# tdavchev/DESIRE

Measured on AMD Instinct MI355X. Metric: agent-trajectory-samples/sec (K=20, T_pred=40), higher is better.
Workload: dtype f32; 1 GPU; BASELINE configs[1]: SDD-like synthetic windows, 32 agent slots/window, K=20, T_obs=8/T_pred=40, H=128, L=128, fp32, posterior CVAE, IOC 1 refinement, social grid 4x4, scene grid 64x64x32; 512 windows/step/GPU; windows_per_gpu=512, rows_per_gpu=327680, parallelism=scene-sharded x1

## Files before the change

### desire_amd/csrc/kernels_conv.hip

```cpp
#include "common.h"
#include "kernels.h"

__global__ __launch_bounds__(DS_WG) void k_conv1(ConvArgs a) {
    __shared__ __attribute__((aligned(16))) float in_s[36 * 40];
    const int n = blockIdx.x, tid = threadIdx.x;
    DYN_N(a, n, n)
    for (int i = tid; i < 36 * 40; i += DS_WG) in_s[i] = 0.f;
    __syncthreads();
    for (int i = tid; i < 1024; i += DS_WG) in_s[((i >> 5) + 1) * 40 + (i & 31) + 1] = a.in[(size_t)n * 1024 + i];
    const int co = tid & 31, pg = tid >> 5;
    float wr[25];
#pragma unroll
    for (int k = 0; k < 25; ++k) wr[k] = a.w_raw[k * 32 + co];
    __syncthreads();
    const float sc = a.scale[co], sh = a.shift[co];
    for (int p = pg; p < 256; p += 8) {
        const int oy = p >> 4, ox = p & 15;
        const int base = (2 * ox) & ~3;
        const bool odd = ox & 1;
        float acc = 0.f;
#pragma unroll
        for (int ky = 0; ky < 5; ++ky) {
            const float* row = in_s + (2 * oy + ky) * 40 + base;
            const float4 v0 = *reinterpret_cast<const float4*>(row), v1 = *reinterpret_cast<const float4*>(row + 4);
            const float t0 = odd ? v0.z : v0.x, t1 = odd ? v0.w : v0.y, t2 = odd ? v1.x : v0.z, t3 = odd ? v1.y : v0.w, t4 = odd ? v1.z : v1.x;
            acc = fmaf(t0, wr[ky * 5 + 0], acc);
            acc = fmaf(t1, wr[ky * 5 + 1], acc);
            acc = fmaf(t2, wr[ky * 5 + 2], acc);
            acc = fmaf(t3, wr[ky * 5 + 3], acc);
            acc = fmaf(t4, wr[ky * 5 + 4], acc);
        }
        { const size_t ix = ((size_t)n * 256 + p) * 32 + co; a.out[ix] = conv_epilogue(acc, sc, sh, a.mode, false, a.yprev, ix); }
    }
}
void launch_conv1(const ConvArgs& a, hipStream_t s) {
    hipLaunchKernelGGL(k_conv1, dim3(a.n), dim3(DS_WG), 0, s, a);
}

template <int CI, int IW, int OW, int STRIDE, int PAD, int CO>
__global__ __launch_bounds__(DS_WG) void k_conv_gather(ConvArgs a) {
    constexpr int PIX = OW * OW, SPW = DS_TM / PIX, LDP = CI + 4, NT = CO / 32, G = CI / 8;
    constexpr int MT = (NT == 4) ? 2 : 1;
    extern __shared__ __attribute__((aligned(16))) float smem[];
    float* zero_row = smem;
    float* in_s = smem + LDP;
    const int lane = lane_id(), w = wave_id(), tid = threadIdx.x;
    const int s0 = blockIdx.x * SPW;
    DYN_N(a, n, s0)
    for (int i = tid; i < LDP; i += DS_WG) zero_row[i] = 0.f;
    constexpr int Q = CI / 4;
    auto pos = [](int y, int x) {
        if (STRIDE == 2) return (((y & 1) * 2 + (x & 1)) * (IW / 2) + (y >> 1)) * (IW / 2) + (x >> 1);
        return y * IW + x;
    };
    for (int i = tid; i < SPW * IW * IW * Q; i += DS_WG) {
        const int pix = i / Q, c4 = i - pix * Q;
        const int ls = pix / (IW * IW), pp = pix - ls * IW * IW;
        const int smp = s0 + ls;
        float4 v = make_float4(0.f, 0.f, 0.f, 0.f);
        if (smp < a.n) v = *reinterpret_cast<const float4*>(a.in + ((size_t)s0 * IW * IW + pix) * CI + c4 * 4);
        *reinterpret_cast<float4*>(in_s + (ls * IW * IW + pos(pp / IW, pp % IW)) * LDP + c4 * 4) = v;
    }
    __syncthreads();
    const int nt = (NT == 4) ? w : (w & 1);
    const int mt0 = (NT == 4) ? 0 : (w >> 1);
    f32x16 acc[MT];
    int oy[MT], ox[MT], sm[MT];
#pragma unroll
    for (int m = 0; m < MT; ++m) {
        acc[m] = zero16();
        const int r = (mt0 + m) * 32 + (lane & 31);
        sm[m] = r / PIX;
        const int q = r - sm[m] * PIX;
        oy[m] = q / OW;
        ox[m] = q - oy[m] * OW;
    }
    for (int ky = 0; ky < 5; ++ky)
        for (int kx = 0; kx < 5; ++kx) {
            const float* ap[MT];
#pragma unroll
            for (int m = 0; m < MT; ++m) {
                const int iy = oy[m] * STRIDE + ky - PAD, ix = ox[m] * STRIDE + kx - PAD;
                const bool ok = iy >= 0 && iy < IW && ix >= 0 && ix < IW;
                ap[m] = (ok ? in_s + (sm[m] * IW * IW + pos(iy, ix)) * LDP : zero_row) + 4 * (lane >> 5);
            }
            mma_groups_ptr<MT>(acc, ap, a.Wp + ((size_t)((ky * 5 + kx) * NT + nt) * G) * 64 + lane, G);
        }
    const int co = nt * 32 + (lane & 31);
    const float sc = a.scale[co], sh = a.shift[co];
#pragma unroll
    for (int m = 0; m < MT; ++m)
#pragma unroll
        for (int i = 0; i < 16; ++i) {
            const int r = (mt0 + m) * 32 + acc_row(i);
            const int smp = s0 + r / PIX;
            if (smp < a.n) { const size_t ix = ((size_t)s0 * PIX + r) * CO + co; a.out[ix] = conv_epilogue(acc[m][i], sc, sh, a.mode, false, a.yprev, ix); }
        }
}
void launch_conv2(const ConvArgs& a, hipStream_t s) {
    const size_t lds = (36 + 256 * 36) * sizeof(float);
    hipLaunchKernelGGL((k_conv_gather<32, 16, 8, 2, 1, 64>), dim3(a.n), dim3(DS_WG), lds, s, a);
}
void launch_conv3(const ConvArgs& a, hipStream_t s) {
    const size_t lds = (68 + 4 * 64 * 68) * sizeof(float);
    launch_big_lds<k_conv_gather<64, 8, 4, 1, 0, 128>>(dim3((a.n + 3) / 4), dim3(DS_WG), lds, s, a);
}

template <bool FWD>
__global__ __launch_bounds__(DS_WG) void k_deconv2(ConvArgs a) {
    extern __shared__ __attribute__((aligned(16))) float out_s[];
    const int lane = lane_id(), w = wave_id();
    const int hf = w & 1, sp = w >> 1;
    asm volatile("" ::: "a255");
    DYN_N(a, n, blockIdx.x * 4)
    for (int bx = blockIdx.x; bx * 4 < a.n; bx += gridDim.x) {
        const int s0 = bx * 4 + sp * 2;
        const int c = lane & 31, hi = lane >> 5;
        float O[8][8];
    #pragma unroll
        for (int oy = 0; oy < 8; ++oy)
    #pragma unroll
            for (int ox = 0; ox < 8; ++ox) O[oy][ox] = 0.f;
        float4 af[16];
        {
            const int row = lane & 31;
            const int smp = min(s0 + ((row >> 2) & 1), a.n - 1);
            const float* src = a.in + ((size_t)smp * 16 + (row >> 3) * 4 + (row & 3)) * 128 + 4 * hi;
    #pragma unroll
            for (int g = 0; g < 16; ++g) af[g] = *reinterpret_cast<const float4*>(src + g * 8);
        }
        int woff = 0;
        asm volatile("" : "+s"(woff));
        const float4* wp = a.Wp + woff + lane;
        auto load_b = [&](float4 (&b)[8], int q) {
            const float4* bp = wp + ((size_t)((q >> 1) * 2 + hf) * 16 + (q & 1) * 8) * 64;
    #pragma unroll
            for (int g = 0; g < 8; ++g) b[g] = bp[g * 64];
        };
        float4 b[2][8];
        load_b(b[0], 0);
        f32x16 acc = zero16();
    #pragma unroll
        for (int q = 0; q < 50; ++q) {
            if (q + 1 < 50) load_b(b[(q + 1) & 1], q + 1);
            __builtin_amdgcn_sched_barrier(0);
            const float4 (&bt)[8] = b[q & 1];
            if (!(q & 1)) acc = zero16();
    #pragma unroll
            for (int g = 0; g < 8; ++g) {
                const float4 av = af[(q & 1) * 8 + g];
                acc = mfma32(av.x, bt[g].x, acc);
                acc = mfma32(av.y, bt[g].y, acc);
                acc = mfma32(av.z, bt[g].z, acc);
                acc = mfma32(av.w, bt[g].w, acc);
            }
            if (q & 1) {
                const int tap = q >> 1, ky = tap / 5, kx = tap - ky * 5;
    #pragma unroll
                for (int i = 0; i < 16; ++i) O[(i >> 2) + ky][(i & 3) + kx] = O[(i >> 2) + ky][(i & 3) + kx] + acc[i];
            }
            __builtin_amdgcn_sched_barrier(0);
        }
        float* my = out_s + (sp * 2) * 4096;
    #pragma unroll
        for (int o = 0; o < 64; ++o) my[(hi * 64 + o) * 64 + hf * 32 + c] = O[o >> 3][o & 7];
        const int er = lane >> 3, ec = hf * 32 + (lane & 7) * 4;
        const float4 sc4 = *reinterpret_cast<const float4*>(a.scale + ec), sh4 = *reinterpret_cast<const float4*>(a.shift + ec);
        for (int i = 0; i < 16; ++i) {
            const int sp_px = i * 8 + er;
            const int smp = s0 + (sp_px >> 6);
            if (smp < a.n) {
                const float4 v = *reinterpret_cast<const float4*>(my + sp_px * 64 + ec);
                const size_t ix = ((size_t)smp * 64 + (sp_px & 63)) * 64 + ec;
                float4 o;
                if (FWD) {
                    o.x = eluf_(v.x * sc4.x + sh4.x); o.y = eluf_(v.y * sc4.y + sh4.y);
                    o.z = eluf_(v.z * sc4.z + sh4.z); o.w = eluf_(v.w * sc4.w + sh4.w);
                } else {
                    o.x = conv_epilogue(v.x, sc4.x, sh4.x, a.mode, false, a.yprev, ix);
                    o.y = conv_epilogue(v.y, sc4.y, sh4.y, a.mode, false, a.yprev, ix + 1);
                    o.z = conv_epilogue(v.z, sc4.z, sh4.z, a.mode, false, a.yprev, ix + 2);
                    o.w = conv_epilogue(v.w, sc4.w, sh4.w, a.mode, false, a.yprev, ix + 3);
                }
                *reinterpret_cast<float4*>(a.out + ix) = o;
            }
        }
    }
}
void launch_deconv2(const ConvArgs& a, hipStream_t s) {
    const int ng = dyn_units(a.n, a.dyn);
    if (a.mode == 0) launch_big_lds<k_deconv2<true>>(dim3((ng + 3) / 4), dim3(DS_WG), 4 * 4096 * sizeof(float), s, a);
    else launch_big_lds<k_deconv2<false>>(dim3((ng + 3) / 4), dim3(DS_WG), 4 * 4096 * sizeof(float), s, a);
}

template <bool FWD, int NS>
__global__ __launch_bounds__(NS * 64) void k_deconv3(ConvArgs a) {
    constexpr int LDP = 68;
    extern __shared__ __attribute__((aligned(16))) float smem[];
    float* zero_row = smem;
    float* in_s = smem + 128;
    const int lane = lane_id(), w = wave_id(), tid = threadIdx.x;
    DYN_N(a, n, blockIdx.x * NS)
    for (int bx = blockIdx.x; bx * NS < a.n; bx += gridDim.x) {
        const int s0 = bx * NS;
        for (int i = tid; i < 128; i += NS * 64) zero_row[i] = 0.f;
        for (int i = tid; i < NS * 64 * 16; i += NS * 64) {
            const int pix = i >> 4, c4 = i & 15;
            const int smp = s0 + (pix >> 6);
            float4 v = make_float4(0.f, 0.f, 0.f, 0.f);
            if (smp < a.n) v = *reinterpret_cast<const float4*>(a.in + ((size_t)s0 * 64 + pix) * 64 + c4 * 4);
            *reinterpret_cast<float4*>(in_s + pix * LDP + c4 * 4) = v;
        }
        __syncthreads();
        const int smp = s0 + w;
        const float* mine = in_s + w * 64 * LDP;
        const int c = lane & 31, hi = lane >> 5;
        float4 sc[4], sh[4];
    #pragma unroll
        for (int q = 0; q < 4; ++q) {
            sc[q] = *reinterpret_cast<const float4*>(a.scale + 8 * q + 4 * hi);
            sh[q] = *reinterpret_cast<const float4*>(a.shift + 8 * q + 4 * hi);
        }
        int qy[2], qx[2];
    #pragma unroll
        for (int m = 0; m < 2; ++m) { const int q = m * 32 + (lane & 31); qy[m] = q >> 3; qx[m] = q & 7; }
        for (int py = 0; py < 2; ++py)
            for (int px = 0; px < 2; ++px) {
                f32x16 acc[2] = {zero16(), zero16()};
                for (int ky = 1 - py; ky < 5; ky += 2)
                    for (int kx = 1 - px; kx < 5; kx += 2) {
                        const int dy = (py + 1 - ky) / 2, dx = (px + 1 - kx) / 2;
                        const float* ap[2];
    #pragma unroll
                        for (int m = 0; m < 2; ++m) {
                            const int iy = qy[m] + dy, ix = qx[m] + dx;
                            const bool ok = iy >= 0 && iy < 8 && ix >= 0 && ix < 8;
                            ap[m] = (ok ? mine + (iy * 8 + ix) * LDP : zero_row + ((((w * 64 + iy * 8 + ix + 64) * LDP + 128) & 63))) + 4 * hi;
                        }
                        mma_groups_ptr<2, true>(acc, ap, a.Wp + ((size_t)(ky * 5 + kx) * 8) * 64 + lane, 8);
                    }
                if (smp < a.n) {
    #pragma unroll
                    for (int m = 0; m < 2; ++m) {
                        const int oy = 2 * qy[m] + py, ox = 2 * qx[m] + px;
                        const size_t base = ((size_t)smp * 256 + oy * 16 + ox) * 32 + 4 * hi;
    #pragma unroll
                        for (int q = 0; q < 4; ++q) {
                            const size_t ix = base + 8 * q;
                            float4 o;
                            if (FWD) {
                                o.x = eluf_(acc[m][4 * q] * sc[q].x + sh[q].x); o.y = eluf_(acc[m][4 * q + 1] * sc[q].y + sh[q].y);
                                o.z = eluf_(acc[m][4 * q + 2] * sc[q].z + sh[q].z); o.w = eluf_(acc[m][4 * q + 3] * sc[q].w + sh[q].w);
                            } else {
                                o.x = conv_epilogue(acc[m][4 * q], sc[q].x, sh[q].x, a.mode, false, a.yprev, ix);
                                o.y = conv_epilogue(acc[m][4 * q + 1], sc[q].y, sh[q].y, a.mode, false, a.yprev, ix + 1);
                                o.z = conv_epilogue(acc[m][4 * q + 2], sc[q].z, sh[q].z, a.mode, false, a.yprev, ix + 2);
                                o.w = conv_epilogue(acc[m][4 * q + 3], sc[q].w, sh[q].w, a.mode, false, a.yprev, ix + 3);
                            }
                            *reinterpret_cast<float4*>(a.out + ix) = o;
                        }
                    }
                }
            }
        __syncthreads();
    }
}
void launch_deconv3(const ConvArgs& a, hipStream_t s) {
    const size_t lds = (128 + (size_t)4 * 64 * 68) * sizeof(float);
    const int ng = dyn_units(a.n, a.dyn);
    if (a.mode == 0) launch_big_lds<k_deconv3<true, 4>>(dim3((ng + 3) / 4), dim3(256), lds, s, a);
    else launch_big_lds<k_deconv3<false, 4>>(dim3((ng + 3) / 4), dim3(256), lds, s, a);
}

__global__ __launch_bounds__(DS_WG) void k_deconv4(ConvArgs a) {
    constexpr int LDP = 36;
    __shared__ __attribute__((aligned(16))) float in_s[256 * LDP];
    __shared__ __attribute__((aligned(16))) float w_s[25 * 32];
    const int n = blockIdx.x, tid = threadIdx.x, lane = lane_id(), w = wave_id();
    for (int i = tid; i < 256 * 8; i += DS_WG) {
        const int pix = i >> 3, c4 = i & 7;
        *reinterpret_cast<float4*>(in_s + pix * LDP + c4 * 4) =
            *reinterpret_cast<const float4*>(a.in + ((size_t)n * 256 + pix) * 32 + c4 * 4);
    }
    for (int i = tid; i < 800; i += DS_WG) w_s[i] = a.w_raw[i];
    __syncthreads();
    const int py = w >> 1, px = w & 1;
    const float sc = a.scale[0], sh = a.shift[0];
    for (int j = 0; j < 4; ++j) {
        const int q = j * 64 + lane;
        const int qy = q >> 4, qx = q & 15;
        float acc = 0.f;
        for (int ky = 1 - py; ky < 5; ky += 2) {
            const int iy = qy + (py + 1 - ky) / 2;
            if (iy < 0 || iy >= 16) continue;
            for (int kx = 1 - px; kx < 5; kx += 2) {
                const int ix = qx + (px + 1 - kx) / 2;
                if (ix < 0 || ix >= 16) continue;
                const float* ip = in_s + (iy * 16 + ix) * LDP;
                const float* wp = w_s + (ky * 5 + kx) * 32;
#pragma unroll
                for (int c4 = 0; c4 < 8; ++c4) {
                    const float4 x = *reinterpret_cast<const float4*>(ip + c4 * 4);
                    const float4 ww = *reinterpret_cast<const float4*>(wp + c4 * 4);
                    acc = fmaf(x.x, ww.x, acc); acc = fmaf(x.y, ww.y, acc);
                    acc = fmaf(x.z, ww.z, acc); acc = fmaf(x.w, ww.w, acc);
                }
            }
        }
        { const size_t ix = (size_t)n * 1024 + (2 * qy + py) * 32 + 2 * qx + px; a.out[ix] = conv_epilogue(acc, sc, sh, a.mode, true, a.yprev, ix); }
    }
}
__global__ __launch_bounds__(DS_WG) void k_deconv4_tp(ConvArgs a) {
    __shared__ float xacc[4 * 1024];
    const int lane = lane_id(), w = wave_id(), tid = threadIdx.x;
    const int smp = blockIdx.x * 4 + w;
    DYN_N(a, n, blockIdx.x * 4)
    for (int i = tid; i < 4 * 1024; i += DS_WG) xacc[i] = 0.f;
    __syncthreads();
    float* xa = xacc + w * 1024;
    const float* __restrict__ wr = a.w_raw;
    if (smp < a.n) {
#pragma unroll 1
        for (int j = 0; j < 4; ++j) {
            const int p = j * 64 + lane, iy = p >> 4, ix = p & 15;
            float4 x[8];
            const float4* src = reinterpret_cast<const float4*>(a.in + ((size_t)smp * 256 + p) * 32);
#pragma unroll
            for (int c4 = 0; c4 < 8; ++c4) x[c4] = src[c4];
#pragma unroll 1
            for (int ky = 0; ky < 5; ++ky) {
                const int Y = 2 * iy + ky - 1;
#pragma unroll
                for (int kx = 0; kx < 5; ++kx) {
                    const float* wt = wr + (ky * 5 + kx) * 32;
                    float acc = 0.f;
#pragma unroll
                    for (int c4 = 0; c4 < 8; ++c4) {
                        acc = fmaf(x[c4].x, wt[c4 * 4], acc); acc = fmaf(x[c4].y, wt[c4 * 4 + 1], acc);
                        acc = fmaf(x[c4].z, wt[c4 * 4 + 2], acc); acc = fmaf(x[c4].w, wt[c4 * 4 + 3], acc);
                    }
                    const int X = 2 * ix + kx - 1;
                    if (Y >= 0 && Y < 32 && X >= 0 && X < 32) xa[Y * 32 + X] += acc;
                }
            }
        }
        const float sc = a.scale[0], sh = a.shift[0];
#pragma unroll
        for (int i = 0; i < 16; ++i) {
            const int o = i * 64 + lane;
            a.out[(size_t)smp * 1024 + o] = sigmoidf_(xa[o] * sc + sh);
        }
    }
}
void launch_deconv4(const ConvArgs& a, hipStream_t s) {
    if (a.mode == 0) hipLaunchKernelGGL(k_deconv4_tp, dim3((a.n + 3) / 4), dim3(DS_WG), 0, s, a);
    else hipLaunchKernelGGL(k_deconv4, dim3(a.n), dim3(DS_WG), 0, s, a);
}
```

### desire_amd/csrc/kernels_rnn.hip

```cpp
#include "common.h"
#include "kernels.h"
#include <cstdlib>
#include <map>
#include <tuple>

#define RNN_WG 512

__device__ __forceinline__ f32x16 splat16(float v) {
    f32x16 z;
#pragma unroll
    for (int i = 0; i < 16; ++i) z[i] = v;
    return z;
}

__device__ __forceinline__ void mma1(f32x16& acc, const float* a_lane, const float4* __restrict__ b_lane, int G) {
    f32x16 t[1] = {acc};
    mma_groups<1>(t, a_lane, 0, b_lane, G);
    acc = t[0];
}

template <int H, int TM, bool ROLL>
__device__ __forceinline__ void encoder_tile(const EncArgs& a, int blk) {
    extern __shared__ __attribute__((aligned(16))) float smem[];
    constexpr int LDH = H + 4, NT = H >> 5, G = H >> 3, NTHR = NT * (TM / 32) * 64;
    float* hs = smem;
    float* xs = smem + TM * LDH;
    const int lane = lane_id(), w = wave_id(), tid = threadIdx.x;
    const int cb = w % NT, mt = w / NT;
    const int A = a.n_scenes * a.mno;
    const int a0 = blk * TM;
    const bool active = cb < NT;
    const int col = cb * 32 + (lane & 31);
    float wr0 = 0, wr1 = 0, wu0 = 0, wu1 = 0, wc0 = 0, wc1 = 0, br = 0, bu = 0, bc = 0;
    if (active) {
        wr0 = a.wx_g[col]; wr1 = a.wx_g[2 * H + col];
        wu0 = a.wx_g[H + col]; wu1 = a.wx_g[2 * H + H + col];
        wc0 = a.wx_c[col]; wc1 = a.wx_c[H + col];
        br = a.b_g[col]; bu = a.b_g[H + col]; bc = a.b_c[col];
    }
    f32x16 h = zero16();
    for (int i = tid; i < TM * LDH; i += NTHR) hs[i] = 0.f;
    const float* a_lane = hs + (mt * 32 + (lane & 31)) * LDH + 4 * (lane >> 5);
    float* my_h = hs + (mt * 32 + 4 * (lane >> 5)) * LDH + col;

    const int n_steps = ROLL ? a.T + a.n_roll : a.T;
    const float* fbase = a.frames;
    float fr0 = 0.f, fr1 = 0.f, fr2 = 0.f;
    if (tid < TM) {
        const int ag = min(a0 + tid, A - 1);
        const int sc = ag / a.mno, slot = ag - sc * a.mno;
        fbase = a.frames + ((size_t)sc * a.T * a.mno + slot) * 3;
        if (a.T > 0) { fr0 = fbase[0]; fr1 = fbase[1]; fr2 = fbase[2]; }
    }
    for (int t = 0; t < n_steps; ++t) {
        if (ROLL && t >= a.T) {
            __syncthreads();
            if (tid < TM) {
                const int ag = min(a0 + tid, A - 1);
                float p5[5];
#pragma unroll
                for (int j = 0; j < 5; ++j) p5[j] = 0.f;
                for (int c = 0; c < H; ++c) {
                    const float hv = hs[tid * LDH + c];
#pragma unroll
                    for (int j = 0; j < 5; ++j) p5[j] = fmaf(hv, a.w5[c * 5 + j], p5[j]);
                }
#pragma unroll
                for (int j = 0; j < 5; ++j) p5[j] += a.b5[j];
                const size_t ix = ((size_t)(t - a.T) * A + ag) * 2;
                const float sdx = expf(p5[2]), sdy = expf(p5[3]), rho = tanhf(p5[4]);
                const float n0 = a.normals[ix], n1 = a.normals[ix + 1];
                const float x = fminf(p5[0] + sdx * n0, 1.0f);
                const float y = fminf(p5[1] + sdy * (rho * n0 + sqrtf(fmaxf(1.0f - rho * rho, 0.f)) * n1), 1.0f);
                xs[tid * 2] = x; xs[tid * 2 + 1] = y;
                if (a0 + tid < A) { a.roll_out[ix] = x; a.roll_out[ix + 1] = y; }
            }
        } else
        if (tid < TM) {
            const int ag = min(a0 + tid, A - 1);
            const float f0 = fr0, f1 = fr1, f2 = fr2;
            if (t + 1 < a.T) { const float* fn = fbase + (size_t)(t + 1) * a.mno * 3; fr0 = fn[0]; fr1 = fn[1]; fr2 = fn[2]; }
            xs[tid * 2 + 0] = __fmul_rn(f1, a.sx);
            xs[tid * 2 + 1] = __fmul_rn(f2, a.sy);
            if (a.sv_x && a0 + tid < A) { a.sv_x[((size_t)ag * a.T + t) * 2] = xs[tid * 2]; a.sv_x[((size_t)ag * a.T + t) * 2 + 1] = xs[tid * 2 + 1]; }
            if (t == a.T - 1 && a0 + tid < A) {
                if (a.p_last) { a.p_last[(size_t)ag * 2] = xs[tid * 2]; a.p_last[(size_t)ag * 2 + 1] = xs[tid * 2 + 1]; }
                if (a.valid) a.valid[ag] = (f0 != 0.f) ? 1 : 0;
            }
        }
        __syncthreads();
        f32x16 rh, u;
        if (active) {
#pragma unroll
            for (int i = 0; i < 16; ++i) {
                const int row = mt * 32 + acc_row(i);
                rh[i] = fmaf(xs[row * 2 + 1], wr1, fmaf(xs[row * 2], wr0, br));
                u[i] = fmaf(xs[row * 2 + 1], wu1, fmaf(xs[row * 2], wu0, bu));
            }
            mma1(rh, a_lane, a.Whg + ((size_t)cb * G) * 64 + lane, G);
            mma1(u, a_lane, a.Whg + ((size_t)(cb + NT) * G) * 64 + lane, G);
#pragma unroll
            for (int i = 0; i < 16; ++i) {
                const float r = sigmoidf_(rh[i]);
                rh[i] = r * h[i]; u[i] = sigmoidf_(u[i]);
                if (a.sv_r) {
                    const int ag = a0 + mt * 32 + acc_row(i);
                    if (ag < A) { const size_t ix = ((size_t)ag * a.T + t) * H + col; a.sv_r[ix] = r; a.sv_u[ix] = u[i]; }
                }
            }
        }
        __syncthreads();
        if (active) {
#pragma unroll
            for (int i = 0; i < 16; ++i) my_h[((i & 3) + 8 * (i >> 2)) * LDH] = rh[i];
        }
        __syncthreads();
        if (active) {
            f32x16 ac;
#pragma unroll
            for (int i = 0; i < 16; ++i) {
                const int row = mt * 32 + acc_row(i);
                ac[i] = fmaf(xs[row * 2 + 1], wc1, fmaf(xs[row * 2], wc0, bc));
            }
            mma1(ac, a_lane, a.Whc + ((size_t)cb * G) * 64 + lane, G);
#pragma unroll
            for (int i = 0; i < 16; ++i) {
                const float c = tanhf_(ac[i]);
                h[i] = gru_blend(u[i], h[i], c);
                if (a.sv_c) {
                    const int ag = a0 + mt * 32 + acc_row(i);
                    if (ag < A) { const size_t ix = ((size_t)ag * a.T + t) * H + col; a.sv_c[ix] = c; a.sv_h[ix] = h[i]; }
                }
            }
        }
        __syncthreads();
        if (active) {
#pragma unroll
            for (int i = 0; i < 16; ++i) my_h[((i & 3) + 8 * (i >> 2)) * LDH] = h[i];
        }
    }
    if (active) {
#pragma unroll
        for (int i = 0; i < 16; ++i) {
            const int ag = a0 + mt * 32 + acc_row(i);
            if (ag < A) a.out[(size_t)ag * a.ldo + col] = h[i];
        }
    }
}
template <int H, int TM, bool ROLL = false>
__global__ __launch_bounds__((H / 32) * (TM / 32) * 64) void k_encoder(EncArgs a) {
    DYN_N(a, mno, blockIdx.x * TM)
    encoder_tile<H, TM, ROLL>(a, blockIdx.x);
}
template <int H, int TM>
__global__ __launch_bounds__((H / 32) * (TM / 32) * 64) void k_encoder_pair(EncArgs a0, EncArgs a1, int nb0) {
    if (a0.dyn.cnt) {
        const int P = __builtin_amdgcn_readfirstlane(a0.dyn.cnt[0]);
        a0.mno = P; a1.mno = P;
        const bool second = (int)blockIdx.x >= nb0;
        for (int blk = second ? (int)blockIdx.x - nb0 : (int)blockIdx.x; blk * TM < P; blk += nb0) {
            if (second) encoder_tile<H, TM, false>(a1, blk); else encoder_tile<H, TM, false>(a0, blk);
            __syncthreads();
        }
        return;
    }
    const int blk = (int)blockIdx.x < nb0 ? (int)blockIdx.x : (int)blockIdx.x - nb0;
    if ((int)blockIdx.x < nb0) encoder_tile<H, TM, false>(a0, blk);
    else encoder_tile<H, TM, false>(a1, blk);
}
void launch_encoder_pair(const EncArgs& a0, const EncArgs& a1, hipStream_t s) {
    constexpr int TM = 32;
    int nb0 = (a0.n_scenes * a0.mno + TM - 1) / TM, nb1 = (a1.n_scenes * a1.mno + TM - 1) / TM;
    if (a0.dyn.cnt) nb0 = nb1 = (dyn_units(a0.n_scenes * a0.mno, a0.dyn) + TM - 1) / TM;
    const size_t lds = (TM * (a0.H + 4) + TM * 2) * sizeof(float);
    const dim3 grid(nb0 + nb1);
    if (a0.H == 256) hipLaunchKernelGGL((k_encoder_pair<256, TM>), grid, dim3(512), lds, s, a0, a1, nb0);
    else if (a0.H == 128) hipLaunchKernelGGL((k_encoder_pair<128, TM>), grid, dim3(256), lds, s, a0, a1, nb0);
    else hipLaunchKernelGGL((k_encoder_pair<64, TM>), grid, dim3(128), lds, s, a0, a1, nb0);
}
void launch_encoder(const EncArgs& a, hipStream_t s) {
    const int A = a.n_scenes * a.mno;
    constexpr int TM = 32;
    const size_t lds = (TM * (a.H + 4) + TM * 2) * sizeof(float);
    const dim3 grid((A + TM - 1) / TM);
    if (a.n_roll > 0) {
        if (a.H == 256) hipLaunchKernelGGL((k_encoder<256, TM, true>), grid, dim3(512), lds, s, a);
        else if (a.H == 128) hipLaunchKernelGGL((k_encoder<128, TM, true>), grid, dim3(256), lds, s, a);
        else hipLaunchKernelGGL((k_encoder<64, TM, true>), grid, dim3(128), lds, s, a);
        return;
    }
    if (a.H == 256) hipLaunchKernelGGL((k_encoder<256, TM>), grid, dim3(512), lds, s, a);
    else if (a.H == 128) hipLaunchKernelGGL((k_encoder<128, TM>), grid, dim3(256), lds, s, a);
    else hipLaunchKernelGGL((k_encoder<64, TM>), grid, dim3(128), lds, s, a);
}

template <int H, int TM, bool SAVE>
__global__ __launch_bounds__((H / 32) * (TM / 32) * 64, 2) void k_decoder(DecArgs a) {
    extern __shared__ __attribute__((aligned(16))) float smem[];
    constexpr int LDH = H + 4, NT = H >> 5, G = H >> 3, NTHR = NT * (TM / 32) * 64, TPR = NTHR / TM;
    float* hs = smem;
    float* xs = smem + TM * LDH;
    float* wo = xs + TM * LDH;
    float* pl = wo + 2 * H;
    const int lane = lane_id(), w = wave_id(), tid = threadIdx.x;
    const int cb = w % NT, mt = w / NT;
    const int row0 = blockIdx.x * TM;
    DYN_P(a, row0)
    const bool active = cb < NT;
    const int col = cb * 32 + (lane & 31);
    for (int i = tid; i < TM * (H >> 2); i += NTHR) {
        const int r = i / (H >> 2), c4 = i - r * (H >> 2);
        const int row = min(row0 + r, a.R - 1);
        *reinterpret_cast<float4*>(xs + r * LDH + c4 * 4) =
            *reinterpret_cast<const float4*>(a.xz + (size_t)row * H + c4 * 4);
        const int ag = agent_of_row(row, a.K, a.mno);
        *reinterpret_cast<float4*>(hs + r * LDH + c4 * 4) =
            *reinterpret_cast<const float4*>(a.Hx + (size_t)ag * a.ldhx + c4 * 4);
    }
    for (int i = tid; i < 2 * H; i += NTHR) wo[i] = a.w_head[i];
    if (tid < TM) {
        const int ag = agent_of_row(min(row0 + tid, a.R - 1), a.K, a.mno);
        pl[tid * 2] = a.p_last[(size_t)ag * 2];
        pl[tid * 2 + 1] = a.p_last[(size_t)ag * 2 + 1];
    }
    __syncthreads();
    const int hq = tid % TPR, hrot = TPR >= 8 ? (hq >> 2) * (TPR == 8 ? 2 : 1) : 0;
    float hw0[16], hw1[16];
#pragma unroll
    for (int jj = 0; jj < 4; ++jj)
#pragma unroll
        for (int e = 0; e < 4; ++e) {
            const int c = hq * 16 + 4 * ((jj + hrot) & 3) + e;
            hw0[4 * jj + e] = wo[c * 2]; hw1[4 * jj + e] = wo[c * 2 + 1];
        }
    const float* x_lane = xs + (mt * 32 + (lane & 31)) * LDH + 4 * (lane >> 5);
    const float* a_lane = hs + (mt * 32 + (lane & 31)) * LDH + 4 * (lane >> 5);
    const float* r_lane = xs + (mt * 32 + (lane & 31)) * LDH + 4 * (lane >> 5);
    float* my_h = hs + (mt * 32 + 4 * (lane >> 5)) * LDH + col;
    float* my_rh = xs + (mt * 32 + 4 * (lane >> 5)) * LDH + col;
    f32x16 xr, xu, xc, h;
    if (active) {
        xr = splat16(a.b_g[col]); xu = splat16(a.b_g[H + col]); xc = splat16(a.b_c[col]);
        mma1(xr, x_lane, a.Wxg + ((size_t)cb * G) * 64 + lane, G);
        mma1(xu, x_lane, a.Wxg + ((size_t)(cb + NT) * G) * 64 + lane, G);
        mma1(xc, x_lane, a.Wxc + ((size_t)cb * G) * 64 + lane, G);
#pragma unroll
        for (int i = 0; i < 16; ++i) h[i] = my_h[((i & 3) + 8 * (i >> 2)) * LDH];
    }
    __syncthreads();
    const float bh0 = a.b_head[0], bh1 = a.b_head[1];
    for (int t = 0; t < a.T; ++t) {
        f32x16 rh, u;
        if (active) {
            rh = xr; u = xu;
            mma1(rh, a_lane, a.Whg + ((size_t)cb * G) * 64 + lane, G);
            mma1(u, a_lane, a.Whg + ((size_t)(cb + NT) * G) * 64 + lane, G);
#pragma unroll
            for (int i = 0; i < 16; ++i) {
                const float r = sigmoidf_(rh[i]);
                rh[i] = r * h[i]; u[i] = sigmoidf_(u[i]);
                if (SAVE && a.sv_r) {
                    const int rl = mt * 32 + acc_row(i);
                    if (row0 + rl < a.R) {
                        const size_t ix = ((size_t)(row0 + rl) * a.T + t) * H + col;
                        a.sv_r[ix] = r; a.sv_u[ix] = u[i];
                    }
                }
            }
#pragma unroll
            for (int i = 0; i < 16; ++i) my_rh[((i & 3) + 8 * (i >> 2)) * LDH] = rh[i];
        }
        __syncthreads();
        if (active) {
            f32x16 ac = xc;
            mma1(ac, r_lane, a.Whc + ((size_t)cb * G) * 64 + lane, G);
#pragma unroll
            for (int i = 0; i < 16; ++i) {
                const float c = tanhf_(ac[i]);
                h[i] = gru_blend(u[i], h[i], c);
                if (SAVE && a.sv_c) {
                    const int rl = mt * 32 + acc_row(i);
                    if (row0 + rl < a.R) a.sv_c[((size_t)(row0 + rl) * a.T + t) * H + col] = c;
                }
            }
#pragma unroll
            for (int i = 0; i < 16; ++i) {
                my_h[((i & 3) + 8 * (i >> 2)) * LDH] = h[i];
                const int rl = mt * 32 + acc_row(i);
                if (SAVE && a.hdump && row0 + rl < a.R) a.hdump[((size_t)(row0 + rl) * a.T + t) * H + col] = h[i];
            }
        }
        __syncthreads();
        {
            const int r = tid / TPR;
            float s0 = 0.f, s1 = 0.f;
#pragma unroll
            for (int jj = 0; jj < 4; ++jj) {
                const float4 hv = *reinterpret_cast<const float4*>(hs + r * LDH + hq * 16 + 4 * ((jj + hrot) & 3));
                s0 = fmaf(hv.x, hw0[4 * jj], s0); s1 = fmaf(hv.x, hw1[4 * jj], s1);
                s0 = fmaf(hv.y, hw0[4 * jj + 1], s0); s1 = fmaf(hv.y, hw1[4 * jj + 1], s1);
                s0 = fmaf(hv.z, hw0[4 * jj + 2], s0); s1 = fmaf(hv.z, hw1[4 * jj + 2], s1);
                s0 = fmaf(hv.w, hw0[4 * jj + 3], s0); s1 = fmaf(hv.w, hw1[4 * jj + 3], s1);
            }
            const int q8 = hq;
            s0 += __shfl_xor(s0, 1); s1 += __shfl_xor(s1, 1);
            s0 += __shfl_xor(s0, 2); s1 += __shfl_xor(s1, 2);
            if (TPR >= 8) { s0 += __shfl_xor(s0, 4); s1 += __shfl_xor(s1, 4); }
            if (TPR >= 16) { s0 += __shfl_xor(s0, 8); s1 += __shfl_xor(s1, 8); }
            if (q8 == 0 && row0 + r < a.R) {
                float2 y = make_float2(pl[r * 2] + (s0 + bh0), pl[r * 2 + 1] + (s1 + bh1));
                *reinterpret_cast<float2*>(a.Y + ((size_t)(row0 + r) * a.T + t) * 2) = y;
            }
        }
    }
}
template <int H, int TM>
static void launch_decoder_t(const DecArgs& a, hipStream_t s) {
    const size_t lds = (2 * TM * (H + 4) + 2 * H + TM * 2) * sizeof(float);
    if (a.sv_r || a.sv_c || a.hdump) {
        launch_big_lds<k_decoder<H, TM, true>>(dim3((a.R + TM - 1) / TM), dim3((H / 32) * (TM / 32) * 64), lds, s, a);
    } else {
        launch_big_lds<k_decoder<H, TM, false>>(dim3((a.R + TM - 1) / TM), dim3((H / 32) * (TM / 32) * 64), lds, s, a);
    }
}
void launch_decoder(const DecArgs& a, hipStream_t s) {
    if (a.H == 256) launch_decoder_t<256, 32>(a, s);
    else if (a.H == 128) {
        launch_decoder_t<128, 32>(a, s);
    }
    else launch_decoder_t<64, 64>(a, s);
}

#include "cluster.h"
#include "ioc_tile.h"
#include "split.h"
template <int TM> struct MaskT { typedef unsigned long long type; };
template <> struct MaskT<32> { typedef unsigned type; };
__device__ __forceinline__ int ffs_(unsigned m) { return __ffs((int)m); }
__device__ __forceinline__ int ffs_(unsigned long long m) { return __ffsll((long long)m); }
typedef float f32x4v __attribute__((ext_vector_type(4)));
template <int G>
__device__ __forceinline__ void ioc_bin_chain(f32x16& acc, const float* a_lane, const float4* __restrict__ b_lane, float4 (&b0)[4]) {
    static_assert(G % 8 == 0, "whole pairs of chunks");
    float4 b1[4];
    float4 an = *reinterpret_cast<const float4*>(a_lane);
    auto chunk = [&](int g0, const float4 (&b)[4]) {
#pragma unroll
        for (int j = 0; j < 4; ++j) {
            const float4 av = an;
            if (g0 + j + 1 < G) an = *reinterpret_cast<const float4*>(a_lane + (g0 + j + 1) * 8);
            __builtin_amdgcn_sched_barrier(0);
            acc = mfma32(av.x, b[j].x, acc);
            acc = mfma32(av.y, b[j].y, acc);
            acc = mfma32(av.z, b[j].z, acc);
            acc = mfma32(av.w, b[j].w, acc);
            __builtin_amdgcn_sched_barrier(0);
        }
    };
#pragma unroll
    for (int c = 0; c < G / 4; c += 2) {
        load_b4(b1, b_lane, 4 * c + 4);
        __builtin_amdgcn_sched_barrier(0);
        chunk(4 * c, b0);
        __builtin_amdgcn_sched_barrier(0);
        if (c + 2 < G / 4) load_b4(b0, b_lane, 4 * c + 8);
        __builtin_amdgcn_sched_barrier(0);
        chunk(4 * c + 4, b1);
        __builtin_amdgcn_sched_barrier(0);
    }
}
template <int H, int EV, int C, int TM, bool TRAIN, bool CP = false, int NSPL = 1, bool PAD = false>
__global__ __launch_bounds__((H / 32) * (TM / 32) * 64, ((H / 32) * (TM / 32) <= 2) ? 1 : 2) void k_ioc(IocArgs a) {
#ifdef DESIRE_IOC_TIMING
    long long tacc[10] = {0, 0, 0, 0, 0, 0, 0, 0, 0, 0};
    long long tprev = clock64();
#endif
    extern __shared__ __attribute__((aligned(16))) float smem[];
    constexpr int NT = H >> 5, E = EV + C + H, KX = E + H, LDX = KX + 4, LDB = H + 4;
    constexpr int NTHR = NT * (TM / 32) * 64, TPR = NTHR / TM;
    constexpr int G8 = KX >> 3, GH = H >> 3;
    constexpr int NCH = H / (4 * TPR);
    const int B = a.G * a.G;
    float* XH = smem;
    float* AB = XH + (TM + 1) * LDX;
    typedef typename MaskT<TM>::type mask_t;
    mask_t* masks = reinterpret_cast<mask_t*>(AB + 2 * TM * LDB);
    float* pc = reinterpret_cast<float*>(masks + TM * B);
    float* pp = pc + TM * 2;
    float* wv = pp + TM * 2;
    float* red = wv + 3 * EV;
    unsigned char* vld = reinterpret_cast<unsigned char*>(red + NT * TM);
    unsigned* occ = reinterpret_cast<unsigned*>(vld + TM);
    unsigned* rowbits = occ + 2;
    unsigned* rowlist = rowbits + 36;
    constexpr IocLds P0 = IocLds::tile(H, EV, C, TM, 0), P1 = IocLds::tile(H, EV, C, TM, 1);
    IOC_LDS_TIED(P0.off(P0.MASKS) == ((TM + 1) * LDX + 2 * TM * LDB) * 4);
    IOC_LDS_TIED(P0.sz[P0.MASKS] == 0 && P1.sz[P1.MASKS] == TM * (int)sizeof(mask_t));
    IOC_LDS_TIED(P0.off(P0.ROWLIST) - P0.off(P0.PC) == (TM * 2 * 2 + 3 * EV + NT * TM) * 4 + TM + (2 + 36) * 4);
    IOC_LDS_TIED(P0.sz[P0.ROWLIST] == 2 * (TM / 4) * 4);

    const int lane = lane_id(), w = wave_id(), tid = threadIdx.x;
    const int cb = w % NT, mt = w / NT;
    const int tile = NSPL > 1 ? (int)blockIdx.x / NSPL : (int)blockIdx.x, member = NSPL > 1 ? (int)blockIdx.x % NSPL : 0;
    const int row0 = tile * TM;
    IOC_DYN(a)
    if (a.dyn.cnt && row0 >= a.R) return;
    unsigned long long my_bins = ~0ull;
    if (NSPL > 1) { my_bins = 0ull; for (int b = member; b < 64; b += NSPL) my_bins |= 1ull << b; }
    const bool active = cb < NT;
    const int col = cb * 32 + (lane & 31);
    const int r8 = tid / TPR, q8 = tid % TPR;
    const int my_row = min(row0 + r8, a.R - 1);
    const int gpt = PAD ? a.gpt : 0;
    const bool dead_row = gpt && (r8 / a.mno >= gpt || tile * gpt + r8 / a.mno >= a.ngrp);
    const int my_scene = gpt ? min(tile * gpt + min(r8 / a.mno, gpt - 1), a.ngrp - 1) / a.K : my_row / (a.K * a.mno);
    const int grp_base = (r8 / a.mno) * a.mno;
    const int my_slot = r8 - grp_base;
    const int n_nb = dead_row ? 0 : a.mno;

    ioc_stage_wv<EV, NTHR>(wv, a.w_vel, a.b_vel, tid);
    for (int i = tid; i < LDX; i += NTHR) XH[TM * LDX + i] = 0.f;
    if (tid < TM) { const int ag = ioc_agent_of_row(min(row0 + tid, a.R - 1), a.K, a.mno, gpt, a.ngrp); vld[tid] = ag >= 0 ? a.valid[ag] : 0; }

    float bgr = 0, bgu = 0, bcc = 0, bso = 0, wsc = 0;
    if (active) { bgr = a.b_g[col]; bgu = a.b_g[H + col]; bcc = a.b_c[col]; bso = a.b_soc[col]; wsc = a.w_score[col]; }
    const float* x_lane = XH + (mt * 32 + (lane & 31)) * LDX + 4 * (lane >> 5);
    float* my_x = XH + (mt * 32 + 4 * (lane >> 5)) * LDX + col;
    const float* grid = a.grids + (size_t)a.grid_of_scene[my_scene] * a.Gh * a.Gw * C;
    const size_t sv_tb = TRAIN ? (size_t)row0 * a.T * H : 0;
    float* sv_r_t = TRAIN ? a.sv_r + sv_tb : nullptr; float* sv_u_t = TRAIN ? a.sv_u + sv_tb : nullptr;
    float* sv_c_t = TRAIN ? a.sv_c + sv_tb : nullptr; float* sv_h_t = TRAIN ? a.sv_h + sv_tb : nullptr;
    auto sv_off = [&](int i, int t) { return (unsigned)(((mt * 32 + 4 * (lane >> 5) + (i & 3) + 8 * (i >> 2)) * a.T + t) * H + col); };

    constexpr int NS = 2;
    auto build = [&](int b, int buf) {
        float* ab = AB + buf * TM * LDB + r8 * LDB;
        mask_t m2 = masks[r8 * B + b];
        int off[NS];
#pragma unroll
        for (int sl = 0; sl < NS; ++sl) {
            off[sl] = m2 ? (grp_base + ffs_(m2) - 1) * LDX : TM * LDX;
            m2 &= m2 - 1;
        }
        float4 s[NCH];
#pragma unroll
        for (int c = 0; c < NCH; ++c) {
            const float4 v0 = *reinterpret_cast<const float4*>(XH + off[0] + E + q8 * 4 + c * 4 * TPR);
            const float4 v1 = *reinterpret_cast<const float4*>(XH + off[1] + E + q8 * 4 + c * 4 * TPR);
            s[c].x = v0.x + v1.x; s[c].y = v0.y + v1.y; s[c].z = v0.z + v1.z; s[c].w = v0.w + v1.w;
        }
        if (__any(m2 != 0)) {
            while (m2) {
                const int j = ffs_(m2) - 1;
                m2 &= m2 - 1;
                const float* src = XH + (grp_base + j) * LDX + E + q8 * 4;
#pragma unroll
                for (int c = 0; c < NCH; ++c) {
                    const float4 v = *reinterpret_cast<const float4*>(src + c * 4 * TPR);
                    s[c].x += v.x; s[c].y += v.y; s[c].z += v.z; s[c].w += v.w;
                }
            }
        }
#pragma unroll
        for (int c = 0; c < NCH; ++c) *reinterpret_cast<float4*>(ab + q8 * 4 + c * 4 * TPR) = s[c];
    };

    for (int it = 0; it < a.iters; ++it) {
        for (int i = tid; i < TM * (H >> 2); i += NTHR) {
            const int r = i / (H >> 2), c4 = i - r * (H >> 2);
            const int ag = ioc_agent_of_row(min(row0 + r, a.R - 1), a.K, a.mno, gpt, a.ngrp);
            *reinterpret_cast<float4*>(XH + r * LDX + E + c4 * 4) =
                ag >= 0 ? *reinterpret_cast<const float4*>(a.Hx + (size_t)ag * a.ldhx + c4 * 4) : make_float4(0.f, 0.f, 0.f, 0.f);
        }
        if (tid < TM) {
            const int ag = ioc_agent_of_row(min(row0 + tid, a.R - 1), a.K, a.mno, gpt, a.ngrp);
            pp[tid * 2] = ag >= 0 ? a.p_last[(size_t)ag * 2] : 0.f;
            pp[tid * 2 + 1] = ag >= 0 ? a.p_last[(size_t)ag * 2 + 1] : 0.f;
        }
        __syncthreads();
        f32x16 h = zero16(), sp = zero16();
        if (active) {
#pragma unroll
            for (int i = 0; i < 16; ++i) h[i] = my_x[((i & 3) + 8 * (i >> 2)) * LDX + E];
        }

        float2 ynext = make_float2(0.f, 0.f);
        if (tid < TM) {
            const float2 y0 = *reinterpret_cast<const float2*>(a.Y + ((size_t)min(row0 + tid, a.R - 1) * a.T) * 2);
            pc[tid * 2] = y0.x; pc[tid * 2 + 1] = y0.y;
        }
        for (int i = tid; i < TM * B; i += NTHR) masks[i] = 0;
        if (tid < 2) occ[tid] = 0;
        if (CP && tid < B) rowbits[tid] = 0;
        __syncthreads();
        const float* rh_lane = AB + (mt * 32 + (lane & 31)) * LDB + 4 * (lane >> 5);
        float* my_rh = AB + (mt * 32 + 4 * (lane >> 5)) * LDB + col;
        constexpr int GX = E >> 3;

        for (int t = 0; t < a.T; ++t) {
            IOC_TICK(0)
            if (tid < TM && t + 1 < a.T)
                ynext = *reinterpret_cast<const float2*>(a.Y + ((size_t)min(row0 + tid, a.R - 1) * a.T + t + 1) * 2);
            {
                const float px = pc[r8 * 2], py = pc[r8 * 2 + 1];
                const float vx = px - pp[r8 * 2], vy = py - pp[r8 * 2 + 1];
                constexpr int per = EV / TPR;
#pragma unroll
                for (int j = q8 * per; j < (q8 + 1) * per; ++j)
                    XH[r8 * LDX + j] = fmaxf(fmaf(vy, wv[EV + j], vx * wv[j]) + wv[2 * EV + j], 0.f);
                int cy, cx;
                scene_cell_dev(px, py, a.Gh, a.Gw, cy, cx);
                const float* gsrc = grid + ((size_t)cy * a.Gw + cx) * C;
                constexpr int cper = C / TPR;
                if (cper >= 4) {
#pragma unroll
                    for (int j = q8 * cper; j < (q8 + 1) * cper; j += 4)
                        *reinterpret_cast<float4*>(XH + r8 * LDX + EV + j) = *reinterpret_cast<const float4*>(gsrc + j);
                } else {
                    *reinterpret_cast<float2*>(XH + r8 * LDX + EV + q8 * 2) = *reinterpret_cast<const float2*>(gsrc + q8 * 2);
                }
                float nbw, nbh;
                nb_opaque(a.nb_w, a.nb_h, nbw, nbh);
                const unsigned long long oc = nb_search<4>(pc, vld, grp_base, n_nb, q8, TPR, my_slot, px, py, nbw, nbh, a.G, a.bin_tab,
                                                          [&](int j, int b) {
                                                              atomicOr(&masks[r8 * B + b], (mask_t)1 << j);
                                                              if (CP) atomicOr(&rowbits[b], 1u << r8);
                                                          });
                nb_publish_occ(oc, occ, B);
                if (CP) {
#pragma unroll
                    for (int c = 0; c < NCH; ++c)
                        *reinterpret_cast<float4*>(XH + r8 * LDX + EV + C + q8 * 4 + c * 4 * TPR) = make_float4(0.f, 0.f, 0.f, 0.f);
                }
            }
            __syncthreads();
            IOC_TICK(1)
            if constexpr (CP) {
                unsigned long long om = ioc_occ64(occ);
                constexpr int T16 = H / 16;
                auto build_c = [&](int b, int buf) {
                    const unsigned rb = rowbits[b];
                    if (!((rb >> r8) & 1u)) return;
                    const int slot = __popc(rb & ((1u << r8) - 1u));
                    float* ab = AB + buf * TM * LDB + slot * LDB;
                    mask_t m2 = masks[r8 * B + b];
                    const int o0 = (grp_base + ffs_(m2) - 1) * LDX;
                    m2 &= m2 - 1;
                    const int o1 = m2 ? (grp_base + ffs_(m2) - 1) * LDX : TM * LDX;
                    m2 &= m2 - 1;
                    float4 sacc[NCH];
#pragma unroll
                    for (int c = 0; c < NCH; ++c) {
                        const float4 v0 = *reinterpret_cast<const float4*>(XH + o0 + E + q8 * 4 + c * 4 * TPR);
                        const float4 v1 = *reinterpret_cast<const float4*>(XH + o1 + E + q8 * 4 + c * 4 * TPR);
                        sacc[c].x = v0.x + v1.x; sacc[c].y = v0.y + v1.y; sacc[c].z = v0.z + v1.z; sacc[c].w = v0.w + v1.w;
                    }
                    while (m2) {
                        const int j = ffs_(m2) - 1;
                        m2 &= m2 - 1;
                        const float* src = XH + (grp_base + j) * LDX + E + q8 * 4;
#pragma unroll
                        for (int c = 0; c < NCH; ++c) {
                            const float4 v = *reinterpret_cast<const float4*>(src + c * 4 * TPR);
                            sacc[c].x += v.x; sacc[c].y += v.y; sacc[c].z += v.z; sacc[c].w += v.w;
                        }
                    }
#pragma unroll
                    for (int c = 0; c < NCH; ++c) *reinterpret_cast<float4*>(ab + q8 * 4 + c * 4 * TPR) = sacc[c];
                    if (q8 == 0) reinterpret_cast<unsigned char*>(rowlist + buf * (TM / 4))[slot] = (unsigned char)r8;
                };
                int buf = 0;
                if (om) build_c(ffs_(om) - 1, 0);
                __syncthreads();
                while (om) {
                    const int b = ffs_(om) - 1;
                    om &= om - 1;
                    const float4* w0 = a.Wsoc_c + ((size_t)(b * T16 + 2 * cb) * T16) * 64 + lane;
                    float4 wf[2][T16];
                    if (active) {
#pragma unroll
                        for (int g = 0; g < T16; ++g) { wf[0][g] = w0[g * 64]; wf[1][g] = w0[(T16 + g) * 64]; }
                    }
                    if (om) build_c(ffs_(om) - 1, buf ^ 1);
                    const int nrows = __popc(__builtin_amdgcn_readfirstlane((int)rowbits[b]));
                    if (active) {
                        for (int c16 = 0; c16 * 16 < nrows; ++c16) {
                            f32x4v a0 = {0.f, 0.f, 0.f, 0.f}, a1 = {0.f, 0.f, 0.f, 0.f};
                            const float* ap = AB + buf * TM * LDB + (16 * c16 + (lane & 15)) * LDB + 4 * (lane >> 4);
#pragma unroll
                            for (int g = 0; g < T16; ++g) {
                                const float4 av = *reinterpret_cast<const float4*>(ap + 16 * g);
                                a0 = __builtin_amdgcn_mfma_f32_16x16x4f32(av.x, wf[0][g].x, a0, 0, 0, 0);
// ... 1103 lines not shown
```

Baseline: 2.506 million samples/s.

## Software-pipeline weight loads in deconv3 and decoder GRU MFMA chains

```diff
diff --git a/desire_amd/csrc/kernels_conv.hip b/desire_amd/csrc/kernels_conv.hip
--- a/desire_amd/csrc/kernels_conv.hip
+++ b/desire_amd/csrc/kernels_conv.hip
@@ -1,5 +1,7 @@
 #include "common.h"
 #include "kernels.h"
+#include <type_traits>
+#include <utility>
 
 __global__ __launch_bounds__(DS_WG) void k_conv1(ConvArgs a) {
     __shared__ __attribute__((aligned(16))) float in_s[36 * 40];
@@ -193,6 +195,16 @@
     else launch_big_lds<k_deconv2<false>>(dim3((ng + 3) / 4), dim3(DS_WG), 4 * 4096 * sizeof(float), s, a);
 }
 
+struct D3Chain { int py, px, ky, kx; bool first, last; };
+__host__ __device__ constexpr D3Chain d3_chain(int s) {
+    const int c = s < 4 ? 0 : s < 10 ? 1 : s < 16 ? 2 : 3, s0 = c == 0 ? 0 : c == 1 ? 4 : c == 2 ? 10 : 16;
+    const int py = c >> 1, px = c & 1, nkx = px ? 3 : 2, n = (py ? 3 : 2) * nkx, i = s - s0;
+    return D3Chain{py, px, 1 - py + 2 * (i / nkx), 1 - px + 2 * (i % nkx), i == 0, i == n - 1};
+}
+template <class F, int... S>
+__device__ __forceinline__ void static_for_(F&& f, std::integer_sequence<int, S...>) { (f(std::integral_constant<int, S>{}), ...); }
+template <int N, class F>
+__device__ __forceinline__ void static_for(F&& f) { static_for_(f, std::make_integer_sequence<int, N>{}); }
 template <bool FWD, int NS>
 __global__ __launch_bounds__(NS * 64) void k_deconv3(ConvArgs a) {
     constexpr int LDP = 68;
@@ -203,6 +215,17 @@
     DYN_N(a, n, blockIdx.x * NS)
     for (int bx = blockIdx.x; bx * NS < a.n; bx += gridDim.x) {
         const int s0 = bx * NS;
+        int woff = 0;
+        asm volatile("" : "+s"(woff));
+        const float4* wp = a.Wp + woff + lane;
+        auto load_b = [&](float4 (&f)[8], const D3Chain ch) __attribute__((always_inline)) {
+            const float4* bp = wp + ((size_t)(ch.ky * 5 + ch.kx) * 8) * 64;
+    #pragma unroll
+            for (int g = 0; g < 8; ++g) f[g] = bp[g * 64];
+        };
+        float4 b[2][8];
+        load_b(b[0], d3_chain(0));
+        __builtin_amdgcn_sched_barrier(0);
         for (int i = tid; i < 128; i += NS * 64) zero_row[i] = 0.f;
         for (int i = tid; i < NS * 64 * 16; i += NS * 64) {
             const int pix = i >> 4, c4 = i & 15;
@@ -213,8 +236,7 @@
         }
         __syncthreads();
         const int smp = s0 + w;
-        const float* mine = in_s + w * 64 * LDP;
-        const int c = lane & 31, hi = lane >> 5;
+        const int hi = lane >> 5;
         float4 sc[4], sh[4];
     #pragma unroll
         for (int q = 0; q < 4; ++q) {
@@ -224,21 +246,39 @@
         int qy[2], qx[2];
     #pragma unroll
         for (int m = 0; m < 2; ++m) { const int q = m * 32 + (lane & 31); qy[m] = q >> 3; qx[m] = q & 7; }
-        for (int py = 0; py < 2; ++py)
-            for (int px = 0; px < 2; ++px) {
-                f32x16 acc[2] = {zero16(), zero16()};
-                for (int ky = 1 - py; ky < 5; ky += 2)
-                    for (int kx = 1 - px; kx < 5; kx += 2) {
-                        const int dy = (py + 1 - ky) / 2, dx = (px + 1 - kx) / 2;
-                        const float* ap[2];
-    #pragma unroll
-                        for (int m = 0; m < 2; ++m) {
-                            const int iy = qy[m] + dy, ix = qx[m] + dx;
-                            const bool ok = iy >= 0 && iy < 8 && ix >= 0 && ix < 8;
-                            ap[m] = (ok ? mine + (iy * 8 + ix) * LDP : zero_row + ((((w * 64 + iy * 8 + ix + 64) * LDP + 128) & 63))) + 4 * hi;
-                        }
-                        mma_groups_ptr<2, true>(acc, ap, a.Wp + ((size_t)(ky * 5 + kx) * 8) * 64 + lane, 8);
-                    }
+        auto rows = [&](const D3Chain ch, const float* (&ap)[2]) __attribute__((always_inline)) {
+            const int dy = (ch.py + 1 - ch.ky) / 2, dx = (ch.px + 1 - ch.kx) / 2;
+    #pragma unroll
+            for (int m = 0; m < 2; ++m) {
+                const int iy = qy[m] + dy, ix = qx[m] + dx;
+                const bool ok = iy >= 0 && iy < 8 && ix >= 0 && ix < 8;
+                const int in_off = 128 + (w * 64 + iy * 8 + ix) * LDP, zero_off = ((w * 64 + iy * 8 + ix + 64) * LDP + 128) & 63;
+                ap[m] = smem + (ok ? in_off : zero_off) + 4 * hi;
+            }
+        };
+        const float* ap[2][2];
+        rows(d3_chain(0), ap[0]);
+        f32x16 acc[2];
+        static_for<25>([&](auto chain_no) __attribute__((always_inline)) {
+            constexpr int s = decltype(chain_no)::value;
+            constexpr D3Chain ch = d3_chain(s);
+            constexpr int py = ch.py, px = ch.px;
+            if constexpr (s + 1 < 25) { load_b(b[(s + 1) & 1], d3_chain(s + 1)); rows(d3_chain(s + 1), ap[(s + 1) & 1]); }
+            __builtin_amdgcn_sched_barrier(0);
+            if constexpr (ch.first) { acc[0] = zero16(); acc[1] = zero16(); }
+            const float4 (&bt)[8] = b[s & 1];
+    #pragma unroll
+            for (int g = 0; g < 8; ++g)
+    #pragma unroll
+                for (int m = 0; m < 2; ++m) {
+                    const float4 av = *reinterpret_cast<const float4*>(ap[s & 1][m] + g * 8);
+                    acc[m] = mfma32(bt[g].x, av.x, acc[m]);
+                    acc[m] = mfma32(bt[g].y, av.y, acc[m]);
+                    acc[m] = mfma32(bt[g].z, av.z, acc[m]);
+                    acc[m] = mfma32(bt[g].w, av.w, acc[m]);
+                    __builtin_amdgcn_sched_barrier(0);
+                }
+            if constexpr (ch.last) {
                 if (smp < a.n) {
     #pragma unroll
                     for (int m = 0; m < 2; ++m) {
@@ -262,6 +302,7 @@
                     }
                 }
             }
+        });
         __syncthreads();
     }
 }
diff --git a/desire_amd/csrc/kernels_rnn.hip b/desire_amd/csrc/kernels_rnn.hip
--- a/desire_amd/csrc/kernels_rnn.hip
+++ b/desire_amd/csrc/kernels_rnn.hip
@@ -194,6 +194,15 @@
     else hipLaunchKernelGGL((k_encoder<64, TM>), grid, dim3(128), lds, s, a);
 }
 
+template <int G>
+__device__ __forceinline__ void ioc_bin_chain(f32x16& acc, const float* a_lane, const float4* __restrict__ b_lane, float4 (&b0)[4]);
+template <int G>
+__device__ __forceinline__ void dec_chain(f32x16& acc, const float* a_lane, const float4* __restrict__ b_lane) {
+    float4 b0[4];
+    load_b4(b0, b_lane, 0);
+    __builtin_amdgcn_sched_barrier(0);
+    ioc_bin_chain<G>(acc, a_lane, b_lane, b0);
+}
 template <int H, int TM, bool SAVE>
 __global__ __launch_bounds__((H / 32) * (TM / 32) * 64, 2) void k_decoder(DecArgs a) {
     extern __shared__ __attribute__((aligned(16))) float smem[];
@@ -241,20 +250,26 @@
     f32x16 xr, xu, xc, h;
     if (active) {
         xr = splat16(a.b_g[col]); xu = splat16(a.b_g[H + col]); xc = splat16(a.b_c[col]);
-        mma1(xr, x_lane, a.Wxg + ((size_t)cb * G) * 64 + lane, G);
-        mma1(xu, x_lane, a.Wxg + ((size_t)(cb + NT) * G) * 64 + lane, G);
-        mma1(xc, x_lane, a.Wxc + ((size_t)cb * G) * 64 + lane, G);
+        dec_chain<G>(xr, x_lane, a.Wxg + ((size_t)cb * G) * 64 + lane);
+        dec_chain<G>(xu, x_lane, a.Wxg + ((size_t)(cb + NT) * G) * 64 + lane);
+        dec_chain<G>(xc, x_lane, a.Wxc + ((size_t)cb * G) * 64 + lane);
 #pragma unroll
         for (int i = 0; i < 16; ++i) h[i] = my_h[((i & 3) + 8 * (i >> 2)) * LDH];
     }
     __syncthreads();
     const float bh0 = a.b_head[0], bh1 = a.b_head[1];
+    const unsigned sv_row = (unsigned)a.T * H, sv_lane0 = (unsigned)(mt * 32 + 4 * (lane >> 5)) * sv_row + col;
     for (int t = 0; t < a.T; ++t) {
         f32x16 rh, u;
+        const size_t sv_t = ((size_t)row0 * a.T + t) * H;
+        unsigned sv_lane = sv_lane0;
+        if (SAVE) asm volatile("" : "+v"(sv_lane));
+        int woff = 0;
+        asm volatile("" : "+s"(woff));
         if (active) {
             rh = xr; u = xu;
-            mma1(rh, a_lane, a.Whg + ((size_t)cb * G) * 64 + lane, G);
-            mma1(u, a_lane, a.Whg + ((size_t)(cb + NT) * G) * 64 + lane, G);
+            dec_chain<G>(rh, a_lane, a.Whg + woff + ((size_t)cb * G) * 64 + lane);
+            dec_chain<G>(u, a_lane, a.Whg + woff + ((size_t)(cb + NT) * G) * 64 + lane);
 #pragma unroll
             for (int i = 0; i < 16; ++i) {
                 const float r = sigmoidf_(rh[i]);
@@ -262,8 +277,8 @@
                 if (SAVE && a.sv_r) {
                     const int rl = mt * 32 + acc_row(i);
                     if (row0 + rl < a.R) {
-                        const size_t ix = ((size_t)(row0 + rl) * a.T + t) * H + col;
-                        a.sv_r[ix] = r; a.sv_u[ix] = u[i];
+                        const unsigned ix = sv_lane + ((i & 3) + 8 * (i >> 2)) * sv_row;
+                        a.sv_r[sv_t + ix] = r; a.sv_u[sv_t + ix] = u[i];
                     }
                 }
             }
@@ -273,21 +288,21 @@
         __syncthreads();
         if (active) {
             f32x16 ac = xc;
-            mma1(ac, r_lane, a.Whc + ((size_t)cb * G) * 64 + lane, G);
+            dec_chain<G>(ac, r_lane, a.Whc + woff + ((size_t)cb * G) * 64 + lane);
 #pragma unroll
             for (int i = 0; i < 16; ++i) {
                 const float c = tanhf_(ac[i]);
                 h[i] = gru_blend(u[i], h[i], c);
                 if (SAVE && a.sv_c) {
                     const int rl = mt * 32 + acc_row(i);
-                    if (row0 + rl < a.R) a.sv_c[((size_t)(row0 + rl) * a.T + t) * H + col] = c;
+                    if (row0 + rl < a.R) a.sv_c[sv_t + (sv_lane + ((i & 3) + 8 * (i >> 2)) * sv_row)] = c;
                 }
             }
 #pragma unroll
             for (int i = 0; i < 16; ++i) {
                 my_h[((i & 3) + 8 * (i >> 2)) * LDH] = h[i];
                 const int rl = mt * 32 + acc_row(i);
-                if (SAVE && a.hdump && row0 + rl < a.R) a.hdump[((size_t)(row0 + rl) * a.T + t) * H + col] = h[i];
+                if (SAVE && a.hdump && row0 + rl < a.R) a.hdump[sv_t + (sv_lane + ((i & 3) + 8 * (i >> 2)) * sv_row)] = h[i];
             }
         }
         __syncthreads();
```

Measured after the change: 2.545 million samples/s, median of 6. +1.6%, better.
